# biter0088/pc-nerf

Measured on AMD Instinct MI355X. Metric: LiDAR rays/s (render+loss) at 128 samples/ray; CD vs ref depth, higher is better.
Workload: dtype fp32 (Linear products: fp16 hi/mid split, 3 MFMA products, fp32 accumulate); 1 GPU; render_rays_train fwd + range/child losses; N_samples=128, N_importance=256, chunk=262144, parallelism=blocks1

## Files before the change

include/pcnerf_hip.h:

```cpp
#ifndef PCNERF_HIP_H
#define PCNERF_HIP_H

#include <stddef.h>
#include <stdint.h>

#ifdef __cplusplus
extern "C" {
#endif

#define PCNERF_ABI_VERSION 1
#define PCNERF_FEATURES 256
#define PCNERF_IN_CH 63

int pcnerf_abi_version(void);
const char* pcnerf_last_error(void);

typedef struct pcnerf_nof_params {
  const float* lin_w[8];
  const float* lin_b[8];
  const float* bn_w[8];
  const float* bn_b[8];
  float* bn_rm[8];
  float* bn_rv[8];
  const float* out_w;
  const float* out_b;
} pcnerf_nof_params;

size_t pcnerf_nof_eval_packed_floats(void);
int pcnerf_nof_pack_eval(const pcnerf_nof_params* params, float* packed, void* stream);

int pcnerf_set_eval_math(int mode);

int pcnerf_nof_query_eval(const float* rays, int64_t n_rays, int ray_stride, const float* z, int n_samples,
                          const float* packed, float* p_out, void* stream);

int pcnerf_nof_forward_eval(const float* emb, int64_t n, const float* packed, float* p_out, void* stream);

int pcnerf_nof_fold_eval(const pcnerf_nof_params* params, double* fold, void* stream);

int pcnerf_nof_query_eval_fold(const float* rays, int64_t n_rays, int ray_stride, const float* z, int n_samples,
                               const double* fold, float* p_out, void* stream);

int pcnerf_nof_forward_eval_fold(const float* emb, int64_t n, const double* fold, float* p_out, void* stream);

int pcnerf_embed(const float* pts, int64_t n, float* out, void* stream);

size_t pcnerf_nof_train_workspace_bytes(int64_t chunk);
int pcnerf_nof_query_train(const float* rays, int64_t n_rays, int ray_stride, const float* z, int n_samples,
                           int64_t chunk, const pcnerf_nof_params* params, float momentum, float eps,
                           void* workspace, size_t workspace_bytes, float* p_out, void* stream);

int pcnerf_set_train_math(int mode);

int pcnerf_set_remat_version(int version);

int pcnerf_nof_forward_train(const float* emb, int64_t n, const pcnerf_nof_params* params, float momentum,
                             float eps, void* workspace, size_t workspace_bytes, float* p_out, void* stream);

typedef struct pcnerf_nof_grads {
  float* lin_w[8];
  float* lin_b[8];
  float* bn_w[8];
  float* bn_b[8];
  float* out_w;
// ... 160 lines not shown
```

pc-nerf_amd/csrc/nof_eval.hip:

```cpp
#include <algorithm>
#include <type_traits>

#include "common.h"
#include "pcnerf_internal.h"
#include "prof.h"

namespace pcn {

constexpr int KG_E = 8, KG_H = 32;
constexpr size_t SZ_E = (size_t)KG_E * 8 * 64 * 4;
constexpr size_t SZ_H = (size_t)KG_H * 8 * 64 * 4;
__host__ __device__ constexpr size_t off_w(int layer, bool epart) {
  return layer == 0 ? 0
       : layer <= 3 ? SZ_E + (size_t)(layer - 1) * SZ_H
       : layer == 4 ? (epart ? SZ_E + 3 * SZ_H : 2 * SZ_E + 3 * SZ_H)
                    : 2 * SZ_E + (size_t)(layer - 1) * SZ_H;
}
constexpr size_t OFF_BIAS = 2 * SZ_E + 7 * SZ_H;
constexpr size_t OFF_WOUT = OFF_BIAS + 8 * 256;
constexpr size_t OFF_BOUT = OFF_WOUT + 256;
constexpr size_t EVAL_F32_FLOATS = OFF_BOUT + 4;
constexpr int EH3_KSTEPS = 60;
constexpr size_t EH_VECS = (size_t)EH3_KSTEPS * 16 * 2 * 64;
constexpr size_t OFF_EH_SW = EVAL_F32_FLOATS;
// ... 183 lines not shown
  const size_t idx = (size_t)blockIdx.x * blockDim.x + threadIdx.x;
  if (idx >= EH_VECS) return;
  const int lane = (int)(idx & 63), part = (int)((idx >> 6) & 1), nb = (int)((idx >> 7) & 15);
  const int gk = (int)(idx >> 11);
  int L = 0;
  while (L < 7 && gk >= eh3_start(L + 1)) ++L;
  const int s0 = gk - eh3_start(L);
  const bool epart = L == 0 || (L == 4 && s0 < 2);
  const int s = L == 4 && !epart ? s0 - 2 : s0;
  const int n = 16 * nb + (lane & 15), g = lane >> 4;
  const int in_f = L == 0 ? 63 : L == 4 ? 319 : 256;
  const float alpha = RAW ? 1.0f : (1.0f / sqrtf(P.bn_rv[L][n] + P.eps)) * P.bn_w[L][n];
  const float sc = ldexpf(1.0f, reinterpret_cast<const int*>(out + OFF_EH_SW)[L]);
  eh_f16x8 v;
#pragma unroll
  for (int e = 0; e < 8; ++e) {
    int col;
    if (epart) {
      const int f = 32 * s + 8 * g + e;
      col = f < 63 ? f : -1;
    } else {
      col = (L == 4 ? 63 : 0) + 32 * s + 16 * (e >> 2) + 4 * g + (e & 3);
    }
    const float w = col < 0 ? 0.0f : (alpha * P.lin_w[L][(size_t)n * in_f + col]) * sc;
    const _Float16 hi = (_Float16)w;
    v[e] = part == 0 ? hi : (_Float16)(w - (float)hi);
  }
  reinterpret_cast<eh_f16x8*>(out + OFF_EH)[idx] = v;
}

constexpr int EH3_SB = 3;
constexpr int EH3_WG_PER_CU = 2;
static_assert(96 % (16 * EH3_SB) == 0, "store_layer_bytes (pcnerf_internal.h) pads a chunk to whole 96-sample blocks");
constexpr int EH3_RING = 2;
template <bool TR, bool ST = false>
__global__ __launch_bounds__(256, EH3_WG_PER_CU) void k_nof_eval_h3(const float* __restrict__ rays, int stride,
                                                        const float* __restrict__ z, int64_t total, int S,
                                                        const float* __restrict__ ein, const float* __restrict__ W,
                                                        float* __restrict__ p_out, const float* __restrict__ coef,
                                                        int64_t chunk, float* __restrict__ hst, int64_t hst_chunk,
                                                        int64_t hst_layer, int cy0) {
  constexpr int SB = EH3_SB, NS = 16 * SB, R3 = EH3_RING, D3 = R3 - 1;
  constexpr bool ORD = TR;
  typedef float f32x4_ __attribute__((ext_vector_type(4)));
  __shared__ eh_f16x8 act[8][SB][2][64];
  __shared__ eh_f16x8 eb[2][SB][2][64];
  __shared__ int sx0s[NS];
  __shared__ __attribute__((aligned(16))) float sbias[(TR ? 16 : 8) * 256];
  __shared__ float emax[NS];
  __shared__ float smax[4][NS];
  __shared__ float pdot[4][NS];
  __shared__ float spos[NS][3];
  __shared__ __attribute__((aligned(16))) float sbraw[TR ? 2 : 1][TR ? 256 : 4];
  const int t = threadIdx.x, w = __builtin_amdgcn_readfirstlane(t >> 6), lane = t & 63, g = lane >> 4, li = lane & 15;
  const int cy = (int)blockIdx.y + cy0;
  const int64_t cb = TR ? (int64_t)cy * chunk : 0;
  const int64_t s0 = cb + (int64_t)blockIdx.x * NS;
  const int64_t send = TR ? (cb + chunk < total ? cb + chunk : total) : total;
  if (s0 >= send) return;
  constexpr bool storing = TR && ST;
  float rz = 0.0f, rr[6] = {};
  if (!ein && t < NS) {
    int64_t gs = s0 + t;
    if (gs >= send) gs = send - 1;
    const float* r = rays + ray_of(gs, S) * stride;
    rz = z[gs];
#pragma unroll
    for (int m = 0; m < 6; ++m) rr[m] = r[m];
  }
  const eh_f16x8* __restrict__ img = reinterpret_cast<const eh_f16x8*>(W + OFF_EH);
  int sw[8];
#pragma unroll
  for (int L = 0; L < 8; ++L) sw[L] = __builtin_amdgcn_readfirstlane(reinterpret_cast<const int*>(W + OFF_EH_SW)[L]);
  int sxB[8];
  if (TR) {
    const int* cs = reinterpret_cast<const int*>(coef + cy * (size_t)TQ_COEF_FLOATS + 16 * 256);
#pragma unroll
    for (int L = 0; L < 8; ++L) sxB[L] = __builtin_amdgcn_readfirstlane(L < 7 ? cs[L] : 0);
  }
  auto load_w = [&](eh_f16x8 (&d)[4][2], int gk) __attribute__((always_inline)) {
    gk = gk < EH3_KSTEPS ? gk : EH3_KSTEPS - 1;
#pragma unroll
    for (int j = 0; j < 4; ++j)
#pragma unroll
      for (int p = 0; p < 2; ++p) d[j][p] = img[((size_t)(gk * 16 + 4 * w + j) * 2 + p) * 64 + lane];
  };
  eh_f16x8 wr[R3][4][2];
#pragma unroll
  for (int k = 0; k < D3; ++k) load_w(wr[k], k);
  if (storing) {
    sbraw[0][t] = W[OFF_BIAS + t];
    sbraw[TR ? 1 : 0][t] = W[OFF_BIAS + 256 + t];
  }
  if (TR) {
    const f32x4_* cf = reinterpret_cast<const f32x4_*>(coef + cy * (size_t)TQ_COEF_FLOATS);
    f32x4_ cv[4];
#pragma unroll
    for (int m = 0; m < 4; ++m) cv[m] = cf[t + 256 * m];
#pragma unroll
    for (int m = 0; m < 4; ++m) {
      const int i = 4 * (t + 256 * m), L = i >> 9, isb = (i >> 8) & 1;
      const int sxo = sxB[L], sxi = (L == 0 || L == 4) ? 0 : sxB[L - 1];
      const int e = isb ? sxo : sxo - sw[L] - sxi;
      reinterpret_cast<f32x4_*>(sbias)[t + 256 * m] =
          f32x4_{ldexpf(cv[m][0], e), ldexpf(cv[m][1], e), ldexpf(cv[m][2], e), ldexpf(cv[m][3], e)};
    }
  } else {
    for (int i = t; i < 8 * 256 / 4; i += 256)
      reinterpret_cast<f32x4_*>(sbias)[i] = reinterpret_cast<const f32x4_*>(W + OFF_BIAS)[i];
  }
  float* const encf = reinterpret_cast<float*>(&act[0][0][0][0]);
  static_assert(sizeof(act) >= NS * 65 * sizeof(float), "encoding staging area");
  if (!ein) {
    if (t < NS) {
      float p[3];
      sample_point(rr, rz, p);
#pragma unroll
      for (int m = 0; m < 3; ++m) {
        spos[t][m] = p[m];
        encf[t * 65 + m] = p[m];
      }
      encf[t * 65 + 63] = 0.0f;
    }
    __syncthreads();
    for (int i = t; i < NS * 30; i += 256) {
      const int sm = i / 30, r = i - 30 * sm, k = r / 3, m = r - 3 * k;
      float sv, cv;
      sincosf((float)(1 << k) * spos[sm][m], &sv, &cv);
      encf[sm * 65 + 3 + 6 * k + m] = sv;
      encf[sm * 65 + 6 + 6 * k + m] = cv;
    }
    __syncthreads();
  }
  if (t < NS) {
    float f[64];
    if (ein) {
      int64_t gs = s0 + t;
      if (gs >= send) gs = send - 1;
#pragma unroll
      for (int k = 0; k < 63; ++k) f[k] = ein[gs * 63 + k];
      f[63] = 0.0f;
    } else {
#pragma unroll
      for (int k = 0; k < 64; ++k) f[k] = encf[t * 65 + k];
    }
    float m = 0.0f;
#pragma unroll
    for (int k = 0; k < 63; ++k) m = fmaxf(m, fabsf(f[k]));
    int sx0 = eh_scale(m);
    if (TR && sxB[3] < sx0) sx0 = sxB[3];
    const float xs = ldexpf(1.0f, sx0);
#pragma unroll
    for (int s = 0; s < 2; ++s)
#pragma unroll
      for (int gg = 0; gg < 4; ++gg) {
        float v[8];
#pragma unroll
        for (int e = 0; e < 8; ++e) v[e] = f[32 * s + 8 * gg + e] * xs;
        eh_f16x8 hi, mid;
        eh_split8(v, hi, mid);
        eb[s][t >> 4][0][(t & 15) + 16 * gg] = hi;
        eb[s][t >> 4][1][(t & 15) + 16 * gg] = mid;
      }
    if (!TR) emax[t] = m;
    sx0s[t] = sx0;
  }
  __syncthreads();
  int sxl[SB];
#pragma unroll
  for (int sb = 0; sb < SB; ++sb) sxl[sb] = sx0s[16 * sb + li];
  f32x4_ acc[4][SB];
  int gk = 0;
  auto kstep_enc = [&](int s, int pos, bool first) __attribute__((always_inline)) {
    load_w(wr[(pos + D3) & (R3 - 1)], gk + D3);
    const eh_f16x8 (&wc)[4][2] = wr[pos & (R3 - 1)];
    eh_f16x8 bh[SB], bm[SB];
#pragma unroll
    for (int sb = 0; sb < SB; ++sb) {
      bh[sb] = eb[s][sb][0][lane];
      bm[sb] = eb[s][sb][1][lane];
      const int d = TR ? 0 : sxl[sb] - sx0s[16 * sb + li];
      if (d != 0) {
        const float xs = ldexpf(1.0f, d);
        float v[8];
#pragma unroll
        for (int e = 0; e < 8; ++e) v[e] = ((float)bh[sb][e] + (float)bm[sb][e]) * xs;
        eh_split8(v, bh[sb], bm[sb]);
      }
    }
#pragma unroll
    for (int o1 = 0; o1 < (ORD ? 4 : SB); ++o1)
#pragma unroll
      for (int o2 = 0; o2 < (ORD ? SB : 4); ++o2) {
        const int sb = ORD ? o2 : o1, j = ORD ? o1 : o2;
        acc[j][sb] = __builtin_amdgcn_mfma_f32_16x16x32_f16(wc[j][0], bm[sb], first ? f32x4_{} : acc[j][sb], 0, 0, 0);
      }
#pragma unroll
    for (int o1 = 0; o1 < (ORD ? 4 : SB); ++o1)
#pragma unroll
      for (int o2 = 0; o2 < (ORD ? SB : 4); ++o2) {
        const int sb = ORD ? o2 : o1, j = ORD ? o1 : o2;
        acc[j][sb] = __builtin_amdgcn_mfma_f32_16x16x32_f16(wc[j][0], bh[sb], acc[j][sb], 0, 0, 0);
      }
#pragma unroll
    for (int o1 = 0; o1 < (ORD ? 4 : SB); ++o1)
#pragma unroll
      for (int o2 = 0; o2 < (ORD ? SB : 4); ++o2) {
        const int sb = ORD ? o2 : o1, j = ORD ? o1 : o2;
        acc[j][sb] = __builtin_amdgcn_mfma_f32_16x16x32_f16(wc[j][1], bh[sb], acc[j][sb], 0, 0, 0);
      }
    ++gk;
  };
  auto hidden_ksteps = [&](int pos0, bool first) __attribute__((always_inline)) {
    eh_f16x8 bh[SB], bm[SB];
#pragma unroll
    for (int sb = 0; sb < SB; ++sb) {
      bm[sb] = act[0][sb][1][lane];
      bh[sb] = act[0][sb][0][lane];
    }
#pragma unroll
    for (int s = 0; s < 8; ++s) {
      const int pos = pos0 + s;
      load_w(wr[(pos + D3) & (R3 - 1)], gk + D3);
      const eh_f16x8 (&wc)[4][2] = wr[pos & (R3 - 1)];
#pragma unroll
      for (int o1 = 0; o1 < (ORD ? 4 : SB); ++o1)
#pragma unroll
        for (int o2 = 0; o2 < (ORD ? SB : 4); ++o2) {
          const int sb = ORD ? o2 : o1, j = ORD ? o1 : o2;
          acc[j][sb] = __builtin_amdgcn_mfma_f32_16x16x32_f16(wc[j][0], bm[sb], (first && s == 0) ? f32x4_{} : acc[j][sb], 0, 0, 0);
        }
      __builtin_amdgcn_sched_barrier(0);
      if (s + 1 < 8) {
#pragma unroll
        for (int sb = 0; sb < SB; ++sb) bm[sb] = act[s + 1][sb][1][lane];
      }
      __builtin_amdgcn_sched_barrier(0);
#pragma unroll
      for (int o1 = 0; o1 < (ORD ? 4 : SB); ++o1)
#pragma unroll
        for (int o2 = 0; o2 < (ORD ? SB : 4); ++o2) {
          const int sb = ORD ? o2 : o1, j = ORD ? o1 : o2;
          acc[j][sb] = __builtin_amdgcn_mfma_f32_16x16x32_f16(wc[j][0], bh[sb], acc[j][sb], 0, 0, 0);
        }
#pragma unroll
      for (int o1 = 0; o1 < (ORD ? 4 : SB); ++o1)
#pragma unroll
        for (int o2 = 0; o2 < (ORD ? SB : 4); ++o2) {
          const int sb = ORD ? o2 : o1, j = ORD ? o1 : o2;
          acc[j][sb] = __builtin_amdgcn_mfma_f32_16x16x32_f16(wc[j][1], bh[sb], acc[j][sb], 0, 0, 0);
        }
      __builtin_amdgcn_sched_barrier(0);
      if (s + 1 < 8) {
#pragma unroll
        for (int sb = 0; sb < SB; ++sb) bh[sb] = act[s + 1][sb][0][lane];
      }
      __builtin_amdgcn_sched_barrier(0);
      ++gk;
    }
  };
  auto epi1 = [&](int L) __attribute__((always_inline)) {
#pragma unroll
    for (int sb = 0; sb < SB; ++sb) {
      const float us = ldexpf(1.0f, -(sw[L] + sxl[sb]));
      float m = 0.0f;
#pragma unroll
      for (int j = 0; j < 4; ++j) {
        const f32x4_ b = *reinterpret_cast<const f32x4_*>(sbias + 256 * L + 64 * w + 16 * j + 4 * g);
#pragma unroll
        for (int q = 0; q < 4; ++q) {
          const float v = __builtin_fmaf(acc[j][sb][q], us, b[q]);
          acc[j][sb][q] = v;
          m = fmaxf(m, fabsf(v));
        }
      }
      m = fmaxf(m, __shfl_xor(m, 16, 64));
      m = fmaxf(m, __shfl_xor(m, 32, 64));
      if (g == 0) smax[w][16 * sb + li] = m;
    }
  };
  auto split_out = [&](const float (&xs)[SB], auto SC) {
#pragma unroll
    for (int sb = 0; sb < SB; ++sb)
#pragma unroll
      for (int jp = 0; jp < 2; ++jp) {
        float v[8];
#pragma unroll
        for (int e = 0; e < 8; ++e) {
          const float a = acc[2 * jp + (e >> 2)][sb][e & 3];
          v[e] = decltype(SC)::value ? a * xs[sb] : a;
        }
        eh_f16x8 hi, mid;
        eh_split8(v, hi, mid);
        act[2 * w + jp][sb][0][lane] = hi;
        act[2 * w + jp][sb][1][lane] = mid;
      }
  };
  auto epi2 = [&](bool with_e) __attribute__((always_inline)) {
    float xs[SB];
#pragma unroll
    for (int sb = 0; sb < SB; ++sb) {
      const int sm = 16 * sb + li;
      float m = fmaxf(fmaxf(smax[0][sm], smax[1][sm]), fmaxf(smax[2][sm], smax[3][sm]));
      if (with_e) m = fmaxf(m, emax[sm]);
      sxl[sb] = eh_scale(m);
      xs[sb] = ldexpf(1.0f, sxl[sb]);
    }
    split_out(xs, std::true_type{});
  };
  auto store_raw = [&](int L, int sb, int j, float sc) __attribute__((always_inline)) {
    const int64_t q = (int64_t)blockIdx.x * SB + sb, tile = q >> 1;
    const int n0 = 64 * w + 16 * j + 4 * g;
    const f32x4_ b = *reinterpret_cast<const f32x4_*>(&sbraw[TR ? L & 1 : 0][TR ? n0 : 0]);
    const f32x4_ v = {acc[j][sb][0] * sc + b[0], acc[j][sb][1] * sc + b[1], acc[j][sb][2] * sc + b[2],
                      acc[j][sb][3] * sc + b[3]};
    const int sl = 16 * (int)(q & 1) + li + 32 * (g & 1);
    char* const hb = reinterpret_cast<char*>(hst + (int64_t)cy * hst_chunk + (int64_t)L * hst_layer);
    const uint32_t off = ((uint32_t)tile * 32u + (uint32_t)(8 * w + (g >> 1))) * 1024u + (uint32_t)sl * 16u +
                         (uint32_t)j * 2048u;
    __builtin_nontemporal_store(v, reinterpret_cast<f32x4_*>(hb + off));
  };
  auto epi_tr = [&](int L, auto PS) __attribute__((always_inline)) {
    constexpr bool ps = decltype(PS)::value;
#pragma unroll
    for (int sb = 0; sb < SB; ++sb) {
      const float us = ps ? ldexpf(1.0f, -sxl[sb]) : 1.0f;
      if (storing) {
        const float sc = ldexpf(1.0f, -(sw[L] + (ps ? sxl[sb] : (L > 0 ? sxB[L - 1] : 0))));
#pragma unroll
        for (int j = 0; j < 4; ++j) store_raw(L, sb, j, sc);
      }
#pragma unroll
      for (int j = 0; j < 4; ++j) {
        const int nb = 64 * w + 16 * j + 4 * g;
        const f32x4_ a = *reinterpret_cast<const f32x4_*>(sbias + 512 * L + nb);
        const f32x4_ b = *reinterpret_cast<const f32x4_*>(sbias + 512 * L + 256 + nb);
#pragma unroll
        for (int q = 0; q < 4; ++q) {
          float v = acc[j][sb][q];
          if (ps) v *= us;
          acc[j][sb][q] = __builtin_fmaf(v, a[q], b[q]);
        }
      }
    }
  };
#pragma unroll
  for (int s = 0; s < 2; ++s) kstep_enc(s, s, s == 0);
  if (TR) {
    epi_tr(0, std::true_type{});
    float xs[SB];
#pragma unroll
    for (int sb = 0; sb < SB; ++sb) {
      sxl[sb] = sxB[0];
      xs[sb] = 1.0f;
    }
    __syncthreads();
    split_out(xs, std::false_type{});
    __syncthreads();
  } else {
    epi1(0);
    __syncthreads();
    epi2(false);
    __syncthreads();
  }
  float bnext = 0.0f;
  auto bias_load = [&](int L) __attribute__((always_inline)) {
    if (storing && L < 7) bnext = W[OFF_BIAS + 256 * (L + 1) + t];
  };
  auto layer_end = [&](int L) __attribute__((always_inline)) {
    if (TR) {
      if (storing && L < 7) sbraw[TR ? (L + 1) & 1 : 0][TR ? t : 0] = bnext;
      if (L == 4) epi_tr(4, std::true_type{});
      else epi_tr(L, std::false_type{});
      if (L < 7) {
        float xs[SB];
#pragma unroll
        for (int sb = 0; sb < SB; ++sb) {
          const int sx0 = sx0s[16 * sb + li];
          sxl[sb] = L == 3 ? sx0 : sxB[L];
          xs[sb] = ldexpf(1.0f, sx0 - sxB[3]);
        }
        __syncthreads();
        if (L == 3) split_out(xs, std::true_type{});
        else split_out(xs, std::false_type{});
        __syncthreads();
      }
    } else {
      epi1(L);
      __syncthreads();
      if (L < 7) {
        epi2(L == 3);
        __syncthreads();
      }
    }
  };
  static_assert(eh3_start(1) % R3 == eh3_start(2) % R3 && eh3_start(2) % R3 == eh3_start(3) % R3, "ring slots");
  static_assert((eh3_start(4) + 2) % R3 == eh3_start(5) % R3 && eh3_start(5) % R3 == eh3_start(6) % R3 &&
                eh3_start(6) % R3 == eh3_start(7) % R3, "ring slots");
#pragma unroll 1
  for (int L = 1; L <= 3; ++L) {
    if (TR) bias_load(L);
    hidden_ksteps(eh3_start(1) % R3, true);
    layer_end(L);
  }
  if (TR) bias_load(4);
#pragma unroll
  for (int s = 0; s < 2; ++s) kstep_enc(s, eh3_start(4) % R3 + s, s == 0);
  hidden_ksteps((eh3_start(4) + 2) % R3, false);
  layer_end(4);
#pragma unroll 1
  for (int L = 5; L <= 7; ++L) {
    if (TR) bias_load(L);
    hidden_ksteps(eh3_start(5) % R3, true);
    layer_end(L);
  }
#pragma unroll
  for (int sb = 0; sb < SB; ++sb) {
    float part = 0.0f;
#pragma unroll
    for (int j = 0; j < 4; ++j) {
      const f32x4_ wv = *reinterpret_cast<const f32x4_*>(W + OFF_WOUT + 64 * w + 16 * j + 4 * g);
#pragma unroll
      for (int q = 0; q < 4; ++q) part = fmaf(wv[q], acc[j][sb][q], part);
    }
    part += __shfl_xor(part, 16, 64);
    part += __shfl_xor(part, 32, 64);
    if (g == 0) pdot[w][16 * sb + li] = part;
  }
  __syncthreads();
  if (t < NS && s0 + t < send) {
    const float logit = ((pdot[0][t] + pdot[1][t]) + (pdot[2][t] + pdot[3][t])) + W[OFF_BOUT];
    p_out[s0 + t] = sigmoid_ref(logit);
  }
}

static int g_eval_math = 1;

static void launch_eval(const float* rays, int stride, const float* z, int64_t total, int S, const float* ein,
                        const float* W, float* p_out, hipStream_t s) {
  if (g_eval_math == 1) {
    const int64_t ns = 16 * EH3_SB;
    hipLaunchKernelGGL(k_nof_eval_h3<false>,
                       dim3((unsigned)((total + ns - 1) / ns)), dim3(256), 0,
                       s, rays, stride, z, total, S, ein, W, p_out, nullptr, (int64_t)0, nullptr, (int64_t)0,
                       (int64_t)0, 0);
  } else {
    const int64_t blocks = ((total + 31) / 32 + 3) / 4;
    hipLaunchKernelGGL(k_nof_eval, dim3((unsigned)blocks), dim3(256), 0, s, rays, stride, z, total, S, ein, W,
                       p_out);
  }
}

__global__ void k_embed(const float* __restrict__ pts, int64_t n, float* __restrict__ out) {
  const int64_t i = (int64_t)blockIdx.x * blockDim.x + threadIdx.x;
  if (i >= n) return;
  const float p[3] = {pts[3 * i], pts[3 * i + 1], pts[3 * i + 2]};
  float e0[32], e1[32];
  encode_half(p, 0, e0);
  encode_half(p, 1, e1);
  float* o = out + 63 * i;
#pragma unroll
  for (int t = 0; t < 32; ++t) {
    o[2 * t] = e0[t];
    if (2 * t + 1 < 63) o[2 * t + 1] = e1[t];
  }
}

__device__ __forceinline__ double gemv_slice(const float* __restrict__ w, int ld, const double* __restrict__ va) {
  double acc[4] = {0.0, 0.0, 0.0, 0.0};
#pragma unroll
  for (int b = 0; b < 64; b += 32) {
    float x[32];
#pragma unroll
    for (int j = 0; j < 32; ++j) x[j] = w[(size_t)(b + j) * ld];
#pragma unroll
    for (int j = 0; j < 32; ++j) acc[j & 3] += va[b + j] * (double)x[j];
  }
  return (acc[0] + acc[1]) + (acc[2] + acc[3]);
// ... 84 lines not shown
        float sv, cv;
        sincosf(sc * p[m], &sv, &cv);
        part[m] += a[3 + 6 * k + m] * (double)sv;
        part[3 + m] += a[6 + 6 * k + m] * (double)cv;
      }
    }
    acc += ((part[0] + part[1]) + (part[2] + part[3])) + (part[4] + part[5]);
  }
  p_out[g] = sigmoid_ref((float)acc);
}

size_t train_query_image_floats() { return EVAL_FLOATS; }

void pack_train_query(const NofParamsDev& P, float* img, hipStream_t s) {
  hipLaunchKernelGGL(k_pack_eval_vectors<true>, dim3(1), dim3(256), 0, s, P, img);
  hipLaunchKernelGGL(k_eval_wscale<true>, dim3(8), dim3(1024), 0, s, P, img);
  hipLaunchKernelGGL(k_pack_eval_h3<true>, dim3((unsigned)((EH_VECS + 255) / 256)),
                     dim3(256), 0, s, P, img);
}

void launch_train_query(const float* rays, int stride, const float* z, int64_t total, int S, const float* ein,
                        const float* img, const float* coef, int64_t chunk, float* p_out, hipStream_t s,
                        float* hst, int64_t hst_chunk, int64_t hst_layer, int64_t store_chunks) {
  const int64_t C = (total + chunk - 1) / chunk;
  const int64_t ns = 16 * EH3_SB;
  const int64_t per = (std::min(chunk, total) + ns - 1) / ns;
  if (C >= 65536 || per >= ((int64_t)1 << 31)) throw std::runtime_error("train query: too many chunks / samples");
  const int64_t Cs = hst ? std::min(store_chunks, C) : 0;
  if (Cs > 0 && hst_layer * sizeof(float) > 0xffffffffull) throw std::runtime_error("train query: store layer >= 4 GiB");
  if (Cs > 0)
    hipLaunchKernelGGL((k_nof_eval_h3<true, true>), dim3((unsigned)per, (unsigned)Cs), dim3(256), 0, s, rays,
                       stride, z, total, S, ein, img, p_out, coef, chunk, hst, hst_chunk, hst_layer, 0);
  if (C > Cs)
    hipLaunchKernelGGL((k_nof_eval_h3<true, false>), dim3((unsigned)per, (unsigned)(C - Cs)), dim3(256), 0, s, rays,
                       stride, z, total, S, ein, img, p_out, coef, chunk, nullptr, (int64_t)0, (int64_t)0, (int)Cs);
}

void launch_fold_logits(const float* rays, int stride, const float* z, int64_t total, int S, const float* ein,
                        const double* fold, int64_t chunk, float* p_out, hipStream_t s) {
  const int64_t blocks = (total + 255) / 256;
  if (blocks >= (int64_t)1 << 31) throw std::runtime_error("fold query: too many samples for one launch");
  const int64_t nfold = (total + chunk - 1) / chunk;
  if (nfold <= 1)
    hipLaunchKernelGGL(k_nof_eval_fold<0>, dim3((unsigned)blocks), dim3(256), 0, s, rays, stride, z, total, S, ein,
                       fold, total, (int64_t)1, p_out);
  else if (chunk >= 256)
    hipLaunchKernelGGL(k_nof_eval_fold<1>, dim3((unsigned)blocks), dim3(256), 0, s, rays, stride, z, total, S, ein,
                       fold, chunk, nfold, p_out);
  else
    hipLaunchKernelGGL(k_nof_eval_fold<2>, dim3((unsigned)blocks), dim3(256), 0, s, rays, stride, z, total, S, ein,
                       fold, chunk, nfold, p_out);
}

}

using namespace pcn;

extern "C" int pcnerf_nof_fold_eval(const pcnerf_nof_params* params, double* fold, void* stream) {
  PCN_API_BEGIN
  PCN_CHECK(params && fold, "pcnerf_nof_fold_eval: null argument");
  NofParamsDev P;
  PCN_CHECK(to_dev_params(params, 1e-5f, &P), "pcnerf_nof_fold_eval: null parameter pointer");
  hipLaunchKernelGGL(k_fold_eval, dim3(1), dim3(1024), 0, (hipStream_t)stream, P, fold);
  PCN_LAUNCH_CHECK("pcnerf_nof_fold_eval");
  PCN_API_END
}

extern "C" int pcnerf_nof_query_eval_fold(const float* rays, int64_t n_rays, int ray_stride, const float* z,
// ... 55 lines not shown

extern "C" int pcnerf_nof_query_eval(const float* rays, int64_t n_rays, int ray_stride, const float* z,
                                     int n_samples, const float* packed, float* p_out, void* stream) {
  PCN_API_BEGIN
  PCN_CHECK(rays && z && packed && p_out, "pcnerf_nof_query_eval: null argument");
  PCN_CHECK(n_rays > 0 && n_samples > 0, "pcnerf_nof_query_eval: empty input");
  PCN_CHECK(ray_stride >= 6, "pcnerf_nof_query_eval: ray_stride < 6");
  const int64_t total = n_rays * (int64_t)n_samples;
  const int64_t tiles = (total + 31) / 32;
  const int64_t blocks = (tiles + 3) / 4;
  PCN_CHECK(blocks < (int64_t)1 << 31, "pcnerf_nof_query_eval: too many samples for one launch");
  {
    ProfScope ps((hipStream_t)stream, PT_EVAL_QUERY, 982528.0 * (double)total,
                 8.0 * (double)total + 4.0 * ray_stride * (double)n_rays + 4.0 * EVAL_F32_FLOATS);
    launch_eval(rays, ray_stride, z, total, n_samples, nullptr, packed, p_out, (hipStream_t)stream);
  }
  PCN_LAUNCH_CHECK("pcnerf_nof_query_eval");
  PCN_API_END
}

extern "C" int pcnerf_nof_forward_eval(const float* emb, int64_t n, const float* packed, float* p_out,
                                       void* stream) {
  PCN_API_BEGIN
  PCN_CHECK(emb && packed && p_out, "pcnerf_nof_forward_eval: null argument");
  PCN_CHECK(n > 0, "pcnerf_nof_forward_eval: empty input");
  const int64_t blocks = ((n + 31) / 32 + 3) / 4;
  PCN_CHECK(blocks < (int64_t)1 << 31, "pcnerf_nof_forward_eval: too many samples for one launch");
  launch_eval(nullptr, 0, nullptr, n, 1, emb, packed, p_out, (hipStream_t)stream);
  PCN_LAUNCH_CHECK("pcnerf_nof_forward_eval");
  PCN_API_END
}


extern "C" int pcnerf_set_eval_math(int mode) {
  if (mode < 0 || mode > 1) {
    pcn::set_error("pcnerf_set_eval_math: mode must be 0 (fp32 MFMA) or 1 (split fp16, 3 products)");
    return -1;
  }
  const int prev = pcn::g_eval_math;
  pcn::g_eval_math = mode;
  return prev;
}
```

pc-nerf_amd/nof/_hip.py:

```python
from __future__ import annotations

import ctypes
import os
import threading

import torch

_HERE = os.path.dirname(os.path.abspath(__file__))
LIB_PATH = os.environ.get("PCNERF_HIP_LIB", os.path.join(os.path.dirname(_HERE), "lib", "libpcnerf_hip.so"))

_lib = None
_lock = threading.Lock()
vp = ctypes.c_void_p
i64 = ctypes.c_int64
c_int = ctypes.c_int
c_float = ctypes.c_float
c_size = ctypes.c_size_t


class NofParams(ctypes.Structure):
    _fields_ = [("lin_w", vp * 8), ("lin_b", vp * 8), ("bn_w", vp * 8), ("bn_b", vp * 8), ("bn_rm", vp * 8),
                ("bn_rv", vp * 8), ("out_w", vp), ("out_b", vp)]


class NofGrads(ctypes.Structure):
    _fields_ = [("lin_w", vp * 8), ("lin_b", vp * 8), ("bn_w", vp * 8), ("bn_b", vp * 8), ("out_w", vp),
                ("out_b", vp)]


_SIGS = {
    "pcnerf_abi_version": (c_int, []),
    "pcnerf_last_error": (ctypes.c_char_p, []),
    "pcnerf_nof_eval_packed_floats": (c_size, []),
    "pcnerf_nof_pack_eval": (c_int, [ctypes.POINTER(NofParams), vp, vp]),
    "pcnerf_nof_query_eval": (c_int, [vp, i64, c_int, vp, c_int, vp, vp, vp]),
    "pcnerf_nof_train_workspace_bytes": (c_size, [i64]),
    "pcnerf_set_train_math": (c_int, [c_int]),
    "pcnerf_set_remat_version": (c_int, [c_int]),
    "pcnerf_set_composite_group": (c_int, [c_int]),
    "pcnerf_set_eval_math": (c_int, [c_int]),
    "pcnerf_nof_query_train": (c_int, [vp, i64, c_int, vp, c_int, i64, ctypes.POINTER(NofParams), c_float, c_float,
                                       vp, c_size, vp, vp]),
    "pcnerf_sample_coarse": (c_int, [vp, i64, c_int, c_int, c_int, c_int, c_int, c_int, c_int, c_int, vp, vp]),
    "pcnerf_perturb": (c_int, [vp, i64, c_int, c_float, vp, vp, vp]),
    "pcnerf_composite": (c_int, [vp, vp, i64, c_int, vp, c_float, c_float, vp, c_int, c_int, c_int, c_int, vp, vp,
                                 vp, vp, vp, vp, vp]),
    "pcnerf_set_depth2_order": (c_int, [c_int]),
    "pcnerf_mean_f64": (c_int, [vp, i64, ctypes.c_double, vp, vp]),
    "pcnerf_resample": (c_int, [vp, vp, i64, c_int, c_int, vp, vp, vp]),
    "pcnerf_sample_pdf": (c_int, [vp, vp, i64, c_int, c_int, vp, vp, vp]),
    "pcnerf_child_loss_workspace_bytes": (c_size, [c_int]),
    "pcnerf_child_loss_reduce": (c_int, [vp, vp, i64, vp, c_int, c_int, vp, vp, vp]),
    "pcnerf_pointwise_loss": (c_int, [vp, vp, vp, i64, c_int, vp, vp]),
    "pcnerf_pointwise_loss_backward": (c_int, [vp, vp, vp, i64, c_int, vp, vp, vp]),
    "pcnerf_child_range_loss_workspace_bytes": (c_size, [c_int]),
    "pcnerf_child_range_loss": (c_int, [vp, vp, i64, vp, c_int, c_int, c_int, c_float, c_float, vp, vp, vp]),
    "pcnerf_child_range_loss_backward": (c_int, [vp, vp, i64, vp, c_int, c_int, c_int, c_float, c_float, vp, vp, vp,
                                                 vp]),
    "pcnerf_embed": (c_int, [vp, i64, vp, vp]),
    "pcnerf_view_rows": (c_int, [vp, vp, i64, c_int, vp, c_int, c_int, c_int, c_int, c_float, vp, c_int, vp, vp, vp,
                                 vp, vp, vp, vp]),
    "pcnerf_view_walk_workspace_bytes": (c_size, [i64]),
    "pcnerf_view_walk": (c_int, [vp, i64, vp, vp, vp, c_int, vp, vp, vp, vp]),
    "pcnerf_rays_workspace_bytes": (c_size, [i64]),
    "pcnerf_build_train_rays": (c_int, [vp, i64, vp, vp, vp, i64, vp, ctypes.c_double, c_int, vp, vp, vp, vp, vp]),
    "pcnerf_count_view_rows": (c_int, [vp, i64, vp, vp, i64, vp, c_int, c_int, vp, vp, vp]),
    "pcnerf_emit_view_rows": (c_int, [vp, i64, vp, vp, i64, vp, c_int, c_int, vp, vp, vp, vp, vp, vp]),
    "pcnerf_child_grid_bytes": (c_size, [i64]),
    "pcnerf_build_child_grid": (c_int, [vp, i64, ctypes.c_double, vp, c_size, vp]),
    "pcnerf_rays_grid_workspace_bytes": (c_size, [i64]),
    "pcnerf_build_train_rays_grid": (c_int, [vp, i64, vp, vp, vp, i64, vp, ctypes.c_double, c_int, vp, vp, vp, vp,
                                             vp, vp]),
    "pcnerf_count_view_rows_grid": (c_int, [vp, i64, vp, vp, i64, vp, c_int, c_int, vp, vp, vp, vp]),
# ... 103 lines not shown
```

pc-nerf_amd/nof/_ops.py:

```python
from __future__ import annotations

import ctypes
import os

import torch

from . import _hip as H

_ws_cache: dict = {}


def _workspace(device: torch.device, nbytes: int) -> torch.Tensor:
    key = (device.type, device.index)
    buf = _ws_cache.get(key)
    if buf is None or buf.numel() < nbytes:
        buf = torch.empty(max(nbytes, 1), dtype=torch.uint8, device=device)
        _ws_cache[key] = buf
    return buf


def _f32(t: torch.Tensor) -> torch.Tensor:
    H.require_device(t)
    if t.dtype != torch.float32:
        t = t.float()
# ... 105 lines not shown
    _TRAIN_FUSED = mode == "f16x2_3_fused"
    return prev_name


def get_train_math() -> str:
    prev = set_train_math("fp32")
    set_train_math(prev)
    return prev


if os.environ.get("PCNERF_TRAIN_MATH"):
    set_train_math(os.environ["PCNERF_TRAIN_MATH"])

EVAL_MATH = {"fp32": 0, "f16x2_3": 1}


def set_eval_math(mode: str) -> str:
    if mode not in EVAL_MATH:
        raise ValueError(f"eval math must be one of {sorted(EVAL_MATH)}")
    prev = H.lib().pcnerf_set_eval_math(EVAL_MATH[mode])
    if prev < 0:
        raise RuntimeError(H.lib().pcnerf_last_error().decode())
    return {v: k for k, v in EVAL_MATH.items()}[prev]


def get_eval_math() -> str:
    prev = set_eval_math("fp32")
    set_eval_math(prev)
    return prev


if os.environ.get("PCNERF_EVAL_MATH"):
    set_eval_math(os.environ["PCNERF_EVAL_MATH"])


_DEPTH2_ORDER = {"stable": 0, "cpu": 1}
_depth2_order = "stable"


def set_depth2_order(order: str) -> str:
    global _depth2_order
    if order not in _DEPTH2_ORDER:
        raise ValueError(f"depth2 order must be one of {sorted(_DEPTH2_ORDER)}")
    H.check(H.lib().pcnerf_set_depth2_order(_DEPTH2_ORDER[order]))
    prev, _depth2_order = _depth2_order, order
    return prev


_TRAIN_FOLD = os.environ.get("PCNERF_TRAIN_FOLD", "0") == "1"


def set_train_fold(enabled: bool) -> bool:
    global _TRAIN_FOLD
    prev, _TRAIN_FOLD = _TRAIN_FOLD, bool(enabled)
    return prev


def train_fold_enabled() -> bool:
    return _TRAIN_FOLD


def fold_state(device, total_samples: int, chunk: int) -> torch.Tensor:
    n = int(H.lib().pcnerf_nof_train_fold_bytes(int(total_samples), int(chunk)))
    return torch.empty((max(n, 1),), dtype=torch.uint8, device=device)


# ... 583 lines not shown
```

Baseline: 782,300 rays/s.

## Add 8-wave wide-tile and deep weight-ring variants of fused MLP query kernel

```diff
diff --git a/include/pcnerf_hip.h b/include/pcnerf_hip.h
--- a/include/pcnerf_hip.h
+++ b/include/pcnerf_hip.h
@@ -30,6 +30,8 @@
 int pcnerf_nof_pack_eval(const pcnerf_nof_params* params, float* packed, void* stream);
 
 int pcnerf_set_eval_math(int mode);
+
+int pcnerf_set_query_geometry(int geometry);
 
 int pcnerf_nof_query_eval(const float* rays, int64_t n_rays, int ray_stride, const float* z, int n_samples,
                           const float* packed, float* p_out, void* stream);
diff --git a/pc-nerf_amd/csrc/nof_eval.hip b/pc-nerf_amd/csrc/nof_eval.hip
--- a/pc-nerf_amd/csrc/nof_eval.hip
+++ b/pc-nerf_amd/csrc/nof_eval.hip
@@ -239,15 +239,20 @@
 constexpr int EH3_SB = 3;
 constexpr int EH3_WG_PER_CU = 2;
 static_assert(96 % (16 * EH3_SB) == 0, "store_layer_bytes (pcnerf_internal.h) pads a chunk to whole 96-sample blocks");
+constexpr int EH3_SB_WIDE = 6;
+static_assert(96 % (16 * EH3_SB_WIDE) == 0, "store_layer_bytes pads a chunk to whole 96-sample blocks");
 constexpr int EH3_RING = 2;
-template <bool TR, bool ST = false>
-__global__ __launch_bounds__(256, EH3_WG_PER_CU) void k_nof_eval_h3(const float* __restrict__ rays, int stride,
+constexpr int EH3_RING_DEEP = 4;
+template <bool TR, bool ST = false, int NW = 4, int SB = EH3_SB, int R3 = EH3_RING>
+__global__ __launch_bounds__(64 * NW, NW == 4 ? EH3_WG_PER_CU : 1) void k_nof_eval_h3(
+                                                        const float* __restrict__ rays, int stride,
                                                         const float* __restrict__ z, int64_t total, int S,
                                                         const float* __restrict__ ein, const float* __restrict__ W,
                                                         float* __restrict__ p_out, const float* __restrict__ coef,
                                                         int64_t chunk, float* __restrict__ hst, int64_t hst_chunk,
                                                         int64_t hst_layer, int cy0) {
-  constexpr int SB = EH3_SB, NS = 16 * SB, R3 = EH3_RING, D3 = R3 - 1;
+  static_assert(NW == 4 || NW == 8, "waves per workgroup");
+  constexpr int NT = 64 * NW, J = 16 / NW, JP = J / 2, WPG = NW / 4, NS = 16 * SB, D3 = R3 - 1;
   constexpr bool ORD = TR;
   typedef float f32x4_ __attribute__((ext_vector_type(4)));
   __shared__ eh_f16x8 act[8][SB][2][64];
@@ -255,7 +260,7 @@
   __shared__ int sx0s[NS];
   __shared__ __attribute__((aligned(16))) float sbias[(TR ? 16 : 8) * 256];
   __shared__ float emax[NS];
-  __shared__ float smax[4][NS];
+  __shared__ float smax[NW][NS];
   __shared__ float pdot[4][NS];
   __shared__ float spos[NS][3];
   __shared__ __attribute__((aligned(16))) float sbraw[TR ? 2 : 1][TR ? 256 : 4];
@@ -285,35 +290,36 @@
 #pragma unroll
     for (int L = 0; L < 8; ++L) sxB[L] = __builtin_amdgcn_readfirstlane(L < 7 ? cs[L] : 0);
   }
-  auto load_w = [&](eh_f16x8 (&d)[4][2], int gk) __attribute__((always_inline)) {
+  auto load_w = [&](eh_f16x8 (&d)[J][2], int gk) __attribute__((always_inline)) {
     gk = gk < EH3_KSTEPS ? gk : EH3_KSTEPS - 1;
 #pragma unroll
-    for (int j = 0; j < 4; ++j)
-#pragma unroll
-      for (int p = 0; p < 2; ++p) d[j][p] = img[((size_t)(gk * 16 + 4 * w + j) * 2 + p) * 64 + lane];
-  };
-  eh_f16x8 wr[R3][4][2];
+    for (int j = 0; j < J; ++j)
+#pragma unroll
+      for (int p = 0; p < 2; ++p) d[j][p] = img[((size_t)(gk * 16 + J * w + j) * 2 + p) * 64 + lane];
+  };
+  eh_f16x8 wr[R3][J][2];
 #pragma unroll
   for (int k = 0; k < D3; ++k) load_w(wr[k], k);
-  if (storing) {
+  if (storing && (NT == 256 || t < 256)) {
     sbraw[0][t] = W[OFF_BIAS + t];
     sbraw[TR ? 1 : 0][t] = W[OFF_BIAS + 256 + t];
   }
   if (TR) {
     const f32x4_* cf = reinterpret_cast<const f32x4_*>(coef + cy * (size_t)TQ_COEF_FLOATS);
-    f32x4_ cv[4];
-#pragma unroll
-    for (int m = 0; m < 4; ++m) cv[m] = cf[t + 256 * m];
-#pragma unroll
-    for (int m = 0; m < 4; ++m) {
-      const int i = 4 * (t + 256 * m), L = i >> 9, isb = (i >> 8) & 1;
+    constexpr int CM = 16 * 256 / 4 / NT;
+    f32x4_ cv[CM];
+#pragma unroll
+    for (int m = 0; m < CM; ++m) cv[m] = cf[t + NT * m];
+#pragma unroll
+    for (int m = 0; m < CM; ++m) {
+      const int i = 4 * (t + NT * m), L = i >> 9, isb = (i >> 8) & 1;
       const int sxo = sxB[L], sxi = (L == 0 || L == 4) ? 0 : sxB[L - 1];
       const int e = isb ? sxo : sxo - sw[L] - sxi;
-      reinterpret_cast<f32x4_*>(sbias)[t + 256 * m] =
+      reinterpret_cast<f32x4_*>(sbias)[t + NT * m] =
           f32x4_{ldexpf(cv[m][0], e), ldexpf(cv[m][1], e), ldexpf(cv[m][2], e), ldexpf(cv[m][3], e)};
     }
   } else {
-    for (int i = t; i < 8 * 256 / 4; i += 256)
+    for (int i = t; i < 8 * 256 / 4; i += NT)
       reinterpret_cast<f32x4_*>(sbias)[i] = reinterpret_cast<const f32x4_*>(W + OFF_BIAS)[i];
   }
   float* const encf = reinterpret_cast<float*>(&act[0][0][0][0]);
@@ -330,7 +336,7 @@
       encf[t * 65 + 63] = 0.0f;
     }
     __syncthreads();
-    for (int i = t; i < NS * 30; i += 256) {
+    for (int i = t; i < NS * 30; i += NT) {
       const int sm = i / 30, r = i - 30 * sm, k = r / 3, m = r - 3 * k;
       float sv, cv;
       sincosf((float)(1 << k) * spos[sm][m], &sv, &cv);
@@ -376,11 +382,11 @@
   int sxl[SB];
 #pragma unroll
   for (int sb = 0; sb < SB; ++sb) sxl[sb] = sx0s[16 * sb + li];
-  f32x4_ acc[4][SB];
+  f32x4_ acc[J][SB];
   int gk = 0;
   auto kstep_enc = [&](int s, int pos, bool first) __attribute__((always_inline)) {
-    load_w(wr[(pos + D3) & (R3 - 1)], gk + D3);
-    const eh_f16x8 (&wc)[4][2] = wr[pos & (R3 - 1)];
+    load_w(wr[(pos + D3) % R3], gk + D3);
+    const eh_f16x8 (&wc)[J][2] = wr[pos % R3];
     eh_f16x8 bh[SB], bm[SB];
 #pragma unroll
     for (int sb = 0; sb < SB; ++sb) {
@@ -396,23 +402,23 @@
       }
     }
 #pragma unroll
-    for (int o1 = 0; o1 < (ORD ? 4 : SB); ++o1)
-#pragma unroll
-      for (int o2 = 0; o2 < (ORD ? SB : 4); ++o2) {
+    for (int o1 = 0; o1 < (ORD ? J : SB); ++o1)
+#pragma unroll
+      for (int o2 = 0; o2 < (ORD ? SB : J); ++o2) {
         const int sb = ORD ? o2 : o1, j = ORD ? o1 : o2;
         acc[j][sb] = __builtin_amdgcn_mfma_f32_16x16x32_f16(wc[j][0], bm[sb], first ? f32x4_{} : acc[j][sb], 0, 0, 0);
       }
 #pragma unroll
-    for (int o1 = 0; o1 < (ORD ? 4 : SB); ++o1)
-#pragma unroll
-      for (int o2 = 0; o2 < (ORD ? SB : 4); ++o2) {
+    for (int o1 = 0; o1 < (ORD ? J : SB); ++o1)
+#pragma unroll
+      for (int o2 = 0; o2 < (ORD ? SB : J); ++o2) {
         const int sb = ORD ? o2 : o1, j = ORD ? o1 : o2;
         acc[j][sb] = __builtin_amdgcn_mfma_f32_16x16x32_f16(wc[j][0], bh[sb], acc[j][sb], 0, 0, 0);
       }
 #pragma unroll
-    for (int o1 = 0; o1 < (ORD ? 4 : SB); ++o1)
-#pragma unroll
-      for (int o2 = 0; o2 < (ORD ? SB : 4); ++o2) {
+    for (int o1 = 0; o1 < (ORD ? J : SB); ++o1)
+#pragma unroll
+      for (int o2 = 0; o2 < (ORD ? SB : J); ++o2) {
         const int sb = ORD ? o2 : o1, j = ORD ? o1 : o2;
         acc[j][sb] = __builtin_amdgcn_mfma_f32_16x16x32_f16(wc[j][1], bh[sb], acc[j][sb], 0, 0, 0);
       }
@@ -428,12 +434,12 @@
 #pragma unroll
     for (int s = 0; s < 8; ++s) {
       const int pos = pos0 + s;
-      load_w(wr[(pos + D3) & (R3 - 1)], gk + D3);
-      const eh_f16x8 (&wc)[4][2] = wr[pos & (R3 - 1)];
-#pragma unroll
-      for (int o1 = 0; o1 < (ORD ? 4 : SB); ++o1)
-#pragma unroll
-        for (int o2 = 0; o2 < (ORD ? SB : 4); ++o2) {
+      load_w(wr[(pos + D3) % R3], gk + D3);
+      const eh_f16x8 (&wc)[J][2] = wr[pos % R3];
+#pragma unroll
+      for (int o1 = 0; o1 < (ORD ? J : SB); ++o1)
+#pragma unroll
+        for (int o2 = 0; o2 < (ORD ? SB : J); ++o2) {
           const int sb = ORD ? o2 : o1, j = ORD ? o1 : o2;
           acc[j][sb] = __builtin_amdgcn_mfma_f32_16x16x32_f16(wc[j][0], bm[sb], (first && s == 0) ? f32x4_{} : acc[j][sb], 0, 0, 0);
         }
@@ -444,16 +450,16 @@
       }
       __builtin_amdgcn_sched_barrier(0);
 #pragma unroll
-      for (int o1 = 0; o1 < (ORD ? 4 : SB); ++o1)
-#pragma unroll
-        for (int o2 = 0; o2 < (ORD ? SB : 4); ++o2) {
+      for (int o1 = 0; o1 < (ORD ? J : SB); ++o1)
+#pragma unroll
+        for (int o2 = 0; o2 < (ORD ? SB : J); ++o2) {
           const int sb = ORD ? o2 : o1, j = ORD ? o1 : o2;
           acc[j][sb] = __builtin_amdgcn_mfma_f32_16x16x32_f16(wc[j][0], bh[sb], acc[j][sb], 0, 0, 0);
         }
 #pragma unroll
-      for (int o1 = 0; o1 < (ORD ? 4 : SB); ++o1)
-#pragma unroll
-        for (int o2 = 0; o2 < (ORD ? SB : 4); ++o2) {
+      for (int o1 = 0; o1 < (ORD ? J : SB); ++o1)
+#pragma unroll
+        for (int o2 = 0; o2 < (ORD ? SB : J); ++o2) {
           const int sb = ORD ? o2 : o1, j = ORD ? o1 : o2;
           acc[j][sb] = __builtin_amdgcn_mfma_f32_16x16x32_f16(wc[j][1], bh[sb], acc[j][sb], 0, 0, 0);
         }
@@ -472,8 +478,8 @@
       const float us = ldexpf(1.0f, -(sw[L] + sxl[sb]));
       float m = 0.0f;
 #pragma unroll
-      for (int j = 0; j < 4; ++j) {
-        const f32x4_ b = *reinterpret_cast<const f32x4_*>(sbias + 256 * L + 64 * w + 16 * j + 4 * g);
+      for (int j = 0; j < J; ++j) {
+        const f32x4_ b = *reinterpret_cast<const f32x4_*>(sbias + 256 * L + 16 * J * w + 16 * j + 4 * g);
 #pragma unroll
         for (int q = 0; q < 4; ++q) {
           const float v = __builtin_fmaf(acc[j][sb][q], us, b[q]);
@@ -490,7 +496,7 @@
 #pragma unroll
     for (int sb = 0; sb < SB; ++sb)
 #pragma unroll
-      for (int jp = 0; jp < 2; ++jp) {
+      for (int jp = 0; jp < JP; ++jp) {
         float v[8];
 #pragma unroll
         for (int e = 0; e < 8; ++e) {
@@ -499,8 +505,8 @@
         }
         eh_f16x8 hi, mid;
         eh_split8(v, hi, mid);
-        act[2 * w + jp][sb][0][lane] = hi;
-        act[2 * w + jp][sb][1][lane] = mid;
+        act[JP * w + jp][sb][0][lane] = hi;
+        act[JP * w + jp][sb][1][lane] = mid;
       }
   };
   auto epi2 = [&](bool with_e) __attribute__((always_inline)) {
@@ -509,6 +515,8 @@
     for (int sb = 0; sb < SB; ++sb) {
       const int sm = 16 * sb + li;
       float m = fmaxf(fmaxf(smax[0][sm], smax[1][sm]), fmaxf(smax[2][sm], smax[3][sm]));
+#pragma unroll
+      for (int k = 4; k < NW; ++k) m = fmaxf(m, smax[k][sm]);
       if (with_e) m = fmaxf(m, emax[sm]);
       sxl[sb] = eh_scale(m);
       xs[sb] = ldexpf(1.0f, sxl[sb]);
@@ -517,13 +525,13 @@
   };
   auto store_raw = [&](int L, int sb, int j, float sc) __attribute__((always_inline)) {
     const int64_t q = (int64_t)blockIdx.x * SB + sb, tile = q >> 1;
-    const int n0 = 64 * w + 16 * j + 4 * g;
+    const int n0 = 16 * J * w + 16 * j + 4 * g;
     const f32x4_ b = *reinterpret_cast<const f32x4_*>(&sbraw[TR ? L & 1 : 0][TR ? n0 : 0]);
     const f32x4_ v = {acc[j][sb][0] * sc + b[0], acc[j][sb][1] * sc + b[1], acc[j][sb][2] * sc + b[2],
                       acc[j][sb][3] * sc + b[3]};
     const int sl = 16 * (int)(q & 1) + li + 32 * (g & 1);
     char* const hb = reinterpret_cast<char*>(hst + (int64_t)cy * hst_chunk + (int64_t)L * hst_layer);
-    const uint32_t off = ((uint32_t)tile * 32u + (uint32_t)(8 * w + (g >> 1))) * 1024u + (uint32_t)sl * 16u +
+    const uint32_t off = ((uint32_t)tile * 32u + (uint32_t)(2 * J * w + (g >> 1))) * 1024u + (uint32_t)sl * 16u +
                          (uint32_t)j * 2048u;
     __builtin_nontemporal_store(v, reinterpret_cast<f32x4_*>(hb + off));
   };
@@ -535,11 +543,11 @@
       if (storing) {
         const float sc = ldexpf(1.0f, -(sw[L] + (ps ? sxl[sb] : (L > 0 ? sxB[L - 1] : 0))));
 #pragma unroll
-        for (int j = 0; j < 4; ++j) store_raw(L, sb, j, sc);
-      }
-#pragma unroll
-      for (int j = 0; j < 4; ++j) {
-        const int nb = 64 * w + 16 * j + 4 * g;
+        for (int j = 0; j < J; ++j) store_raw(L, sb, j, sc);
+      }
+#pragma unroll
+      for (int j = 0; j < J; ++j) {
+        const int nb = 16 * J * w + 16 * j + 4 * g;
         const f32x4_ a = *reinterpret_cast<const f32x4_*>(sbias + 512 * L + nb);
         const f32x4_ b = *reinterpret_cast<const f32x4_*>(sbias + 512 * L + 256 + nb);
 #pragma unroll
@@ -572,11 +580,11 @@
   }
   float bnext = 0.0f;
   auto bias_load = [&](int L) __attribute__((always_inline)) {
-    if (storing && L < 7) bnext = W[OFF_BIAS + 256 * (L + 1) + t];
+    if (storing && L < 7 && (NT == 256 || t < 256)) bnext = W[OFF_BIAS + 256 * (L + 1) + t];
   };
   auto layer_end = [&](int L) __attribute__((always_inline)) {
     if (TR) {
-      if (storing && L < 7) sbraw[TR ? (L + 1) & 1 : 0][TR ? t : 0] = bnext;
+      if (storing && L < 7 && (NT == 256 || t < 256)) sbraw[TR ? (L + 1) & 1 : 0][TR ? t : 0] = bnext;
       if (L == 4) epi_tr(4, std::true_type{});
       else epi_tr(L, std::false_type{});
       if (L < 7) {
@@ -621,18 +629,32 @@
     hidden_ksteps(eh3_start(5) % R3, true);
     layer_end(L);
   }
-#pragma unroll
-  for (int sb = 0; sb < SB; ++sb) {
-    float part = 0.0f;
-#pragma unroll
-    for (int j = 0; j < 4; ++j) {
-      const f32x4_ wv = *reinterpret_cast<const f32x4_*>(W + OFF_WOUT + 64 * w + 16 * j + 4 * g);
+  auto occ_chain = [&](int sb, float part) __attribute__((always_inline)) {
+#pragma unroll
+    for (int j = 0; j < J; ++j) {
+      const f32x4_ wv = *reinterpret_cast<const f32x4_*>(W + OFF_WOUT + 16 * J * w + 16 * j + 4 * g);
 #pragma unroll
       for (int q = 0; q < 4; ++q) part = fmaf(wv[q], acc[j][sb][q], part);
     }
-    part += __shfl_xor(part, 16, 64);
-    part += __shfl_xor(part, 32, 64);
-    if (g == 0) pdot[w][16 * sb + li] = part;
+    return part;
+  };
+  float (*const hand)[SB][64] = reinterpret_cast<float (*)[SB][64]>(&eb[0][0][0][0]);
+  static_assert(sizeof(eb) >= 4 * SB * 64 * sizeof(float), "occ_out handover area");
+  if (WPG == 2) {
+    if (!(w & 1)) {
+#pragma unroll
+      for (int sb = 0; sb < SB; ++sb) hand[w >> 1][sb][lane] = occ_chain(sb, 0.0f);
+    }
+    __syncthreads();
+  }
+  if (WPG == 1 || (w & 1)) {
+#pragma unroll
+    for (int sb = 0; sb < SB; ++sb) {
+      float part = occ_chain(sb, WPG == 1 ? 0.0f : hand[w >> 1][sb][lane]);
+      part += __shfl_xor(part, 16, 64);
+      part += __shfl_xor(part, 32, 64);
+      if (g == 0) pdot[w / WPG][16 * sb + li] = part;
+    }
   }
   __syncthreads();
   if (t < NS && s0 + t < send) {
@@ -643,14 +665,29 @@
 
 static int g_eval_math = 1;
 
+static int g_query_geometry = -1;
+constexpr int EH3_GEOM_EVAL = 0, EH3_GEOM_TRAIN = 1;
+
+template <bool TR, typename... Args>
+static void launch_h3(int geom, int64_t span, unsigned rows, hipStream_t s, Args... args) {
+  const bool wide = geom & 1, deep = geom & 2;
+  const int64_t ns = 16 * (wide ? EH3_SB_WIDE : EH3_SB);
+  const dim3 grid((unsigned)((span + ns - 1) / ns), rows), block(wide ? 512 : 256);
+  if (wide && deep)
+    hipLaunchKernelGGL((k_nof_eval_h3<TR, false, 8, EH3_SB_WIDE, EH3_RING_DEEP>), grid, block, 0, s, args...);
+  else if (wide)
+    hipLaunchKernelGGL((k_nof_eval_h3<TR, false, 8, EH3_SB_WIDE, EH3_RING>), grid, block, 0, s, args...);
+  else if (deep)
+    hipLaunchKernelGGL((k_nof_eval_h3<TR, false, 4, EH3_SB, EH3_RING_DEEP>), grid, block, 0, s, args...);
+  else
+    hipLaunchKernelGGL((k_nof_eval_h3<TR, false, 4, EH3_SB, EH3_RING>), grid, block, 0, s, args...);
+}
+
 static void launch_eval(const float* rays, int stride, const float* z, int64_t total, int S, const float* ein,
                         const float* W, float* p_out, hipStream_t s) {
   if (g_eval_math == 1) {
-    const int64_t ns = 16 * EH3_SB;
-    hipLaunchKernelGGL(k_nof_eval_h3<false>,
-                       dim3((unsigned)((total + ns - 1) / ns)), dim3(256), 0,
-                       s, rays, stride, z, total, S, ein, W, p_out, nullptr, (int64_t)0, nullptr, (int64_t)0,
-                       (int64_t)0, 0);
+    launch_h3<false>(g_query_geometry < 0 ? EH3_GEOM_EVAL : g_query_geometry, total, 1u, s, rays, stride, z, total, S,
+                     ein, W, p_out, (const float*)nullptr, (int64_t)0, (float*)nullptr, (int64_t)0, (int64_t)0, 0);
   } else {
     const int64_t blocks = ((total + 31) / 32 + 3) / 4;
     hipLaunchKernelGGL(k_nof_eval, dim3((unsigned)blocks), dim3(256), 0, s, rays, stride, z, total, S, ein, W,
@@ -801,8 +838,9 @@
     hipLaunchKernelGGL((k_nof_eval_h3<true, true>), dim3((unsigned)per, (unsigned)Cs), dim3(256), 0, s, rays,
                        stride, z, total, S, ein, img, p_out, coef, chunk, hst, hst_chunk, hst_layer, 0);
   if (C > Cs)
-    hipLaunchKernelGGL((k_nof_eval_h3<true, false>), dim3((unsigned)per, (unsigned)(C - Cs)), dim3(256), 0, s, rays,
-                       stride, z, total, S, ein, img, p_out, coef, chunk, nullptr, (int64_t)0, (int64_t)0, (int)Cs);
+    launch_h3<true>(g_query_geometry < 0 ? EH3_GEOM_TRAIN : g_query_geometry, std::min(chunk, total),
+                    (unsigned)(C - Cs), s, rays, stride, z, total, S, ein, img, p_out, coef, chunk, (float*)nullptr,
+                    (int64_t)0, (int64_t)0, (int)Cs);
 }
 
 void launch_fold_logits(const float* rays, int stride, const float* z, int64_t total, int S, const float* ein,
@@ -924,6 +962,17 @@
 }
 
 
+extern "C" int pcnerf_set_query_geometry(int geometry) {
+  if (geometry < -1 || geometry > 3) {
+    pcn::set_error("pcnerf_set_query_geometry: geometry must be -1 (default) or 0..3 (bit 0: 8-wave workgroup, "
+                   "bit 1: 4-slot weight ring)");
+    return -2;
+  }
+  const int prev = pcn::g_query_geometry;
+  pcn::g_query_geometry = geometry;
+  return prev;
+}
+
 extern "C" int pcnerf_set_eval_math(int mode) {
   if (mode < 0 || mode > 1) {
     pcn::set_error("pcnerf_set_eval_math: mode must be 0 (fp32 MFMA) or 1 (split fp16, 3 products)");
diff --git a/pc-nerf_amd/nof/_hip.py b/pc-nerf_amd/nof/_hip.py
--- a/pc-nerf_amd/nof/_hip.py
+++ b/pc-nerf_amd/nof/_hip.py
@@ -39,6 +39,7 @@
     "pcnerf_set_remat_version": (c_int, [c_int]),
     "pcnerf_set_composite_group": (c_int, [c_int]),
     "pcnerf_set_eval_math": (c_int, [c_int]),
+    "pcnerf_set_query_geometry": (c_int, [c_int]),
     "pcnerf_nof_query_train": (c_int, [vp, i64, c_int, vp, c_int, i64, ctypes.POINTER(NofParams), c_float, c_float,
                                        vp, c_size, vp, vp]),
     "pcnerf_sample_coarse": (c_int, [vp, i64, c_int, c_int, c_int, c_int, c_int, c_int, c_int, c_int, vp, vp]),
diff --git a/pc-nerf_amd/nof/_ops.py b/pc-nerf_amd/nof/_ops.py
--- a/pc-nerf_amd/nof/_ops.py
+++ b/pc-nerf_amd/nof/_ops.py
@@ -161,6 +161,17 @@
 
 if os.environ.get("PCNERF_EVAL_MATH"):
     set_eval_math(os.environ["PCNERF_EVAL_MATH"])
+
+
+def set_query_geometry(geometry: int) -> int:
+    prev = H.lib().pcnerf_set_query_geometry(int(geometry))
+    if prev < -1:
+        raise ValueError(H.lib().pcnerf_last_error().decode())
+    return prev
+
+
+if os.environ.get("PCNERF_QUERY_GEOMETRY"):
+    set_query_geometry(int(os.environ["PCNERF_QUERY_GEOMETRY"]))
 
 
 _DEPTH2_ORDER = {"stable": 0, "cpu": 1}
```

Result: faster. 815,700 rays/s, median of 6 (+4.3%).
